# yellofi/SelectiveNet_for_semantic_segmentation_binary

Measured on AMD Instinct MI355X. Metric: train images/sec, SelectiveUNet_B 256x256 bs=128 (global), selective_loss s_lamb=2, higher is better.
Workload: dtype f32; 1 GPU; SelectiveUNet_B train step, global bs=128, 256x256, Adam lr=1e-3, s_lamb=2; model=SelectiveUNet_B, global_batch=128, per_gpu_batch=128, image=256, parallelism=dp1

## Files before the change

### selectivenet_for_semantic_segmentation_binary_amd/csrc/conv3x3.hip

```cpp
#include <cstdlib>

#include "gemm_common.h"

namespace selunet {

constexpr int TH = 16, TW = 16;
constexpr int HHT = TH + 2, HWT = TW + 2;
constexpr int HPIX = HHT * HWT;
constexpr int HTHREADS = 512;
constexpr int A_ROUNDS = (HPIX * 8 + HTHREADS - 1) / HTHREADS;
constexpr int AROWB = 160;
__device__ __forceinline__ int halo_off(int hp, int cc) { return hp * AROWB + ((cc ^ ((hp / HWT) & 1)) << 4); }

template <typename T, int BN, bool ONE_CHUNK>
__global__ void __launch_bounds__(HTHREADS, ONE_CHUNK ? 2 : 1)
conv3x3_halo_kernel(GatherArg g, const T* __restrict__ B, int N, int k_pad, EpiArg ep, int n_tiles, int tiles_x,
                    int tiles_y) {
  constexpr int E = 16 / sizeof(T);
  constexpr int CK = 128 / sizeof(T);
  constexpr int WAVES_N = BN / 64;
  constexpr int WAVES_M = 8 / WAVES_N;
  constexpr int WPIX = (TH * TW) / WAVES_M;
  constexpr int MT = WPIX / 32;
  constexpr int NT = 2;
// ... 133 lines not shown
  b_store(rb_next, 0);
  rb_next = b_load(nsteps > 1 ? 1 : 0);
  __syncthreads();

  if constexpr (ONE_CHUNK) {
#pragma unroll
    for (int t = 0; t < 9; ++t) {
      BRegs rb_far = rb_next;
      if (t + 2 < 9) rb_far = b_load(t + 2);
      mma_step(0, t & 1, t);
      if (t + 1 < 9) b_store(rb_next, (t + 1) & 1);
      __syncthreads();
      rb_next = rb_far;
    }
  } else {
    uint4 ra[A_ROUNDS];
    for (int c = 0; c < nchunks; ++c) {
      const int cn = c + 1 < nchunks ? c + 1 : c;
      int cs = cn * CK;
      const bool s1 = g.nsrc > 1 && cs >= g.src[0].C;
      if (s1) cs -= g.src[0].C;
      const SrcArg sn = pick_src(g, s1 ? 1 : 0);
      float* ssc = Ss + ((c + 1) & 1) * CK;
      float* ssh = Ss + 2 * CK + ((c + 1) & 1) * CK;
      float coef = 0.0f;
#pragma unroll
      for (int t = 0; t < 9; ++t) {
        const int s = c * 9 + t;
        const BRegs rb_far = b_load(s + 2 < nsteps ? s + 2 : nsteps - 1);
        if (t == 0 && sn.scale && tid < 2 * CK) coef = tid < CK ? sn.scale[cs + tid] : sn.shift[cs + tid - CK];
        if (t < A_ROUNDS) {
          int hp, cc;
          a_slot(t, hp, cc);
          ra[t] = *a_ptr(cn, hp, cc);
        }
        mma_step(c & 1, s & 1, t);
        b_store(rb_next, (s + 1) & 1);
        if (t == 1 && sn.scale && tid < 2 * CK) (tid < CK ? ssc[tid] : ssh[tid - CK]) = coef;
        if (t >= AD && t - AD < A_ROUNDS) {
          const int r = t - AD;
          int hp, cc;
          if (a_slot(r, hp, cc)) {
            uint4 v = make_uint4(0, 0, 0, 0);
            if (a_inside(hp)) {
              v = ra[r];
              if (sn.scale) {
                T e[E];
                __builtin_memcpy(e, &v, 16);
#pragma unroll
                for (int j = 0; j < E; ++j) {
                  float f = to_f(e[j]) * ssc[cc * E + j] + ssh[cc * E + j];
                  if (sn.relu) f = fmaxf(f, 0.0f);
                  e[j] = from_f<T>(f);
                }
                __builtin_memcpy(&v, e, 16);
              }
            }
            *reinterpret_cast<uint4*>(As + ((c + 1) & 1) * HPIX * AROWB + halo_off(hp, cc)) = v;
          }
        }
        __syncthreads();
        rb_next = rb_far;
      }
    }
  }

  float* tile = reinterpret_cast<float*>(smem);
  acc_to_lds<MT, NT, BN>(tile, acc, wm * WPIX, wn * 64, lane);
  __syncthreads();
  auto dst = [&](int pix, int c) -> T* {
    const int y = y0 + pix / TW, x = x0 + pix % TW;
    if (y >= g.h || x >= g.w) return nullptr;
    const int64_t m = ((int64_t)img * g.h + y) * g.w + x;
    const int col = n0 + c;
    if (ep.mode == SELUNET_EP_SPLIT)
      return col < ep.split ? reinterpret_cast<T*>(ep.out0) + m * ep.split + col
                            : reinterpret_cast<T*>(ep.out1) + m * (N - ep.split) + (col - ep.split);
    return reinterpret_cast<T*>(ep.out0) + m * N + col;
  };
  auto bias_col = [&](int c) { return n0 + c; };
  lds_tile_store<T, TH * TW, BN, HTHREADS>(tile, tid, dst, ep.bias, bias_col, tile_stats(ep, ptile, n0, N));
}

template <typename T, int BN, bool X2, bool M16 = false, bool TQ = false>
__global__ void __launch_bounds__(HTHREADS, 1)
conv3x3_halo_persist_kernel(GatherArg g, const T* __restrict__ B, int N, int k_pad, EpiArg ep, int n_tiles,
                            int tiles_x, int tiles_y, int ptiles, int gp, const float* __restrict__ wcs,
                            const float* __restrict__ amax0, const float* __restrict__ amax1,
                            unsigned* __restrict__ tq = nullptr) {
  static_assert(!TQ || X2, "tile queue: split-fp16 kernel only");
  static_assert(!X2 || std::is_same<T, float>::value, "split-fp16 form of fp32 operands only");
  static_assert(!M16 || X2, "16x16x32 form: split-fp16 only (the bf16 form lost every A/B, retired in round 6)");
  constexpr int E = 16 / sizeof(T);
  constexpr int CK = 128 / sizeof(T);
  constexpr int WAVES_N = BN / 64;
  constexpr int WAVES_M = 8 / WAVES_N;
  constexpr int WPIX = (TH * TW) / WAVES_M;
  constexpr int MT = WPIX / 32;
  constexpr int NT = 2;
  constexpr int RT = WPIX / 16;
  using AccT = std::conditional_t<M16, f32x4, f32x16>;
  constexpr int AM = M16 ? RT : MT, AN = M16 ? 4 : NT;
  constexpr int WROWB = M16 ? 160 : ROWB;
  constexpr int B_ROUNDS = BN * 8 / HTHREADS;
  static_assert(B_ROUNDS * HTHREADS == BN * 8, "weight tile rows must split evenly over the threads");
  auto halo_load_tap = [](int r) { return r; };
  auto halo_write_tap = [](int r) { return r + 3; };
  static_assert(A_ROUNDS <= 6, "halo slice schedule covers six slices");

  constexpr int SMEM_MAIN = 2 * HPIX * AROWB + 2 * BN * WROWB + 2 * CK * 8;
  constexpr int SMEM_EPI = TH * TW * (BN + 4) * 4;
  __shared__ __attribute__((aligned(16))) unsigned char smem[SMEM_MAIN > SMEM_EPI ? SMEM_MAIN : SMEM_EPI];
  unsigned char* As = smem;
  unsigned char* Bs = smem + 2 * HPIX * AROWB;
  float* Ss = reinterpret_cast<float*>(Bs + 2 * BN * WROWB);

  const int tid = threadIdx.x;
  const int lane = tid & 63, wave = tid >> 6;
  const int wm = wave / WAVES_N, wn = wave % WAVES_N;
  const int half = lane >> 5, l32 = lane & 31;
  const int l16 = lane & 15, kg = lane >> 4;

  const unsigned lb = xcd_remap(blockIdx.x, gridDim.x);
  const int n_tile = lb % n_tiles;
  const int prow = lb / n_tiles;
  const int n0 = n_tile * BN;
  const int nchunks = g.Ctot / CK;
  const int ntl = TQ ? 0 : (prow < ptiles ? (ptiles - prow + gp - 1) / gp : 0);
  __shared__ int tq_slot;
  int pt_cur = 0, pt_next = 0;
  if constexpr (TQ) {
    if (tid == 0) tq_slot = (int)min(atomicAdd(tq + n_tile, 1u), (unsigned)ptiles);
    __syncthreads();
    pt_cur = tq_slot;
  }
  const int csteps = nchunks * 9;
  float xs = 1.0f;
  float cfac[AN] = {};
  if constexpr (X2) {
    float am = amax0 ? amax0[0] : 0.0f;
    if (g.nsrc > 1 && amax1) am = fmaxf(am, amax1[0]);
    float inv;
    xs = x2_scale(am, &inv);
#pragma unroll
    for (int b = 0; b < AN; ++b)
      cfac[b] = wcs[n0 + wn * 64 + (M16 ? b * 16 + l16 : b * 32 + l32)] * inv;
  }
  auto halo_store = [&](int hb, int hp, int cc, uint4 v) __attribute__((always_inline)) {
    unsigned char* base = As + hb * HPIX * AROWB + hp * AROWB;
    if constexpr (X2) {
      float f[4];
      __builtin_memcpy(f, &v, 16);
      f16x4 h, l;
#pragma unroll
      for (int e = 0; e < 4; ++e) {
        _Float16 a, b;
        x2_split(f[e] * xs, a, b);
        h[e] = a;
        l[e] = b;
      }
      const int par = (hp / HWT) & 1;
      *reinterpret_cast<f16x4*>(base + (((cc >> 1) ^ par) << 4) + (cc & 1) * 8) = h;
      *reinterpret_cast<f16x4*>(base + (((4 + (cc >> 1)) ^ par) << 4) + (cc & 1) * 8) = l;
    } else {
      *reinterpret_cast<uint4*>(base + (((cc ^ ((hp / HWT) & 1))) << 4)) = v;
    }
  };

  auto halo_store_prepped = [&](int hb, int hp, int cc, uint4 v) __attribute__((always_inline)) {
    unsigned char* base = As + hb * HPIX * AROWB + hp * AROWB;
    if constexpr (X2) {
      const int par = (hp / HWT) & 1;
      *reinterpret_cast<uint2*>(base + (((cc >> 1) ^ par) << 4) + (cc & 1) * 8) = make_uint2(v.x, v.y);
      *reinterpret_cast<uint2*>(base + (((4 + (cc >> 1)) ^ par) << 4) + (cc & 1) * 8) = make_uint2(v.z, v.w);
    } else {
      *reinterpret_cast<uint4*>(base + (((cc ^ ((hp / HWT) & 1))) << 4)) = v;
    }
  };
  auto tile_xy = [&](int pt_i, int& img, int& y0, int& x0) __attribute__((always_inline)) {
    const unsigned pt = (unsigned)pt_i;
    const unsigned r = pt / (unsigned)tiles_x;
    x0 = (int)(pt - r * (unsigned)tiles_x) * TW;
    const unsigned r2 = r / (unsigned)tiles_y;
    y0 = (int)(r - r2 * (unsigned)tiles_y) * TH;
    img = (int)r2;
  };
  auto a_slot = [&](int round, int& hp, int& cc) -> bool {
    const int hidx = round * HTHREADS + tid;
    hp = min(hidx >> 3, HPIX - 1);
    cc = hidx & 7;
    return hidx < HPIX * 8;
  };
  auto a_inside = [&](int y0, int x0, int hp) -> bool {
    const int hy = hp / HWT, hx = hp - (hp / HWT) * HWT;
    return (unsigned)(y0 - 1 + hy) < (unsigned)g.h && (unsigned)(x0 - 1 + hx) < (unsigned)g.w;
  };
  auto chunk_src = [&](int chunk, int& c) -> SrcArg {
    c = chunk * CK;
    const bool s1 = g.nsrc > 1 && c >= g.src[0].C;
    if (s1) c -= g.src[0].C;
    return pick_src(g, s1 ? 1 : 0);
  };
  auto a_ptr = [&](const SrcArg& sa, int c, int img, int y0, int x0, int hp, int cc) -> const uint4* {
    const int hy = hp / HWT, hx = hp - (hp / HWT) * HWT;
    const int ys = min(max(y0 - 1 + hy, 0), g.h - 1), xs = min(max(x0 - 1 + hx, 0), g.w - 1);
    return reinterpret_cast<const uint4*>(reinterpret_cast<const T*>(sa.data) +
                                          (((int64_t)img * g.h + ys) * g.w + xs) * sa.C + c + cc * E);
  };
  constexpr int XRPIX = 3 * HWT;
  static_assert(!X2 || (A_ROUNDS * 3 == HHT && XRPIX * 8 <= HTHREADS), "three halo rows per round");
  const int xq = tid >> 3, xcc = tid & 7;
  const int xhp = xq < XRPIX ? xq : xq - XRPIX;
  const int xry = (xhp >= HWT) + (xhp >= 2 * HWT), xhx = xhp - xry * HWT;
  const unsigned xpix = (unsigned)(xry * g.w + xhx);
  const unsigned xb_off = (unsigned)(xq * k_pad * 4 + xcc * 16);
  const unsigned xb_rstride = (unsigned)(64 * k_pad * 4);
  auto x_lds = [](int t) __attribute__((always_inline)) {
    const int q = t >> 3, cc = t & 7, hp = q < XRPIX ? q : q - XRPIX;
    const int ry = (hp >= HWT) + (hp >= 2 * HWT);
    return (unsigned)(hp * AROWB + (((cc >> 1) ^ (ry & 1)) << 4) + (cc & 1) * 8);
  };
  const unsigned xlds = x_lds(tid);
  unsigned xtb = 0;
  if constexpr (X2) {
    const int hrem = g.h - (tiles_y - 1) * TH, wrem = g.w - (tiles_x - 1) * TW;
#pragma unroll
    for (int r = 0; r < A_ROUNDS; ++r) {
      const int hy = 3 * r + xry;
      xtb |= (unsigned)((hy == 0) | (hy > hrem) << 6 | (xhx == 0) << 12 | (xhx > wrem) << 18) << r;
// ... 140 lines not shown
#pragma unroll
      for (int ks = 0; ks < 2; ++ks) {
        f16x8 ah[MT], al[MT], bh[NT], bl[NT];
#pragma unroll
        for (int a = 0; a < MT; ++a) {
          const unsigned char* p = a_src + (hrow0[a] + tap_off) * AROWB + ((hsw0[a] ^ dy) & 1) * 16;
          ah[a] = *reinterpret_cast<const f16x8*>(p + ks * 32);
          al[a] = *reinterpret_cast<const f16x8*>(p + (2 + ks) * 32);
        }
#pragma unroll
        for (int b = 0; b < NT; ++b) {
          const unsigned char* p = b_src + (wn * 64 + b * 32 + l32) * ROWB + half * 16;
          bh[b] = *reinterpret_cast<const f16x8*>(p + ks * 32);
          bl[b] = *reinterpret_cast<const f16x8*>(p + (2 + ks) * 32);
        }
#pragma unroll
        for (int a = 0; a < MT; ++a)
#pragma unroll
          for (int b = 0; b < NT; ++b) {
            acc[a][b] = __builtin_amdgcn_mfma_f32_32x32x16_f16(ah[a], bl[b], acc[a][b], 0, 0, 0);
            acc[a][b] = __builtin_amdgcn_mfma_f32_32x32x16_f16(al[a], bh[b], acc[a][b], 0, 0, 0);
            acc[a][b] = __builtin_amdgcn_mfma_f32_32x32x16_f16(ah[a], bh[b], acc[a][b], 0, 0, 0);
          }
      }
    } else {
#pragma unroll
      for (int q = 0; q < 4; ++q) {
        const int boff = q * 32 + half * 16;
        uint4 af[MT], bfr[NT];
#pragma unroll
        for (int a = 0; a < MT; ++a)
          af[a] = *reinterpret_cast<const uint4*>(a_src + (hrow0[a] + tap_off) * AROWB + q * 32 + ((hsw0[a] ^ dy) & 1) * 16);
#pragma unroll
        for (int b = 0; b < NT; ++b)
          bfr[b] = *reinterpret_cast<const uint4*>(b_src + (wn * 64 + b * 32 + l32) * WROWB + boff);
#pragma unroll
        for (int a = 0; a < MT; ++a)
#pragma unroll
          for (int b = 0; b < NT; ++b) Mma<T>::run(acc[a][b], af[a], bfr[b]);
      }
    }
  };
  auto halo_put_global = [&](uint4 v, int r, const SrcArg& sa, int c, int y0, int x0, int hb)
      __attribute__((always_inline)) {
    int hp, cc;
    if (!a_slot(r, hp, cc)) return;
    uint4 o = make_uint4(0, 0, 0, 0);
    if (a_inside(y0, x0, hp)) o = sa.scale ? transform16<T>(v, sa.scale, sa.shift, c + cc * E, sa.relu) : v;
    halo_store(hb, hp, cc, o);
  };

  Geo gc{}, gn{};
  if constexpr (X2) gc = gn = tile_geo(TQ ? pt_cur : prow);
  if (!TQ || pt_cur < ptiles) {
    int c0;
    const SrcArg sa = chunk_src(0, c0);
    uint4 v0[A_ROUNDS];
    if constexpr (X2) {
      const XStage s0 = x_stage(gc, sa, c0);
#pragma unroll
      for (int r = 0; r < A_ROUNDS; ++r) v0[r] = x_load(s0, sa, r);
#pragma unroll
      for (int r = 0; r < A_ROUNDS; ++r) {
        uint4 o = make_uint4(0, 0, 0, 0);
        if (!x_out(s0, r)) o = sa.scale ? transform16<T>(v0[r], sa.scale, sa.shift, c0 + xcc * E, sa.relu) : v0[r];
        x_put(0, r, xlds, x_split4(o));
      }
    } else {
      int img, y0, x0;
      tile_xy(TQ ? pt_cur : prow, img, y0, x0);
#pragma unroll
      for (int r = 0; r < A_ROUNDS; ++r) {
        int hp, cc;
        a_slot(r, hp, cc);
        v0[r] = *a_ptr(sa, c0, img, y0, x0, hp, cc);
      }
#pragma unroll
      for (int r = 0; r < A_ROUNDS; ++r) halo_put_global(v0[r], r, sa, c0, y0, x0, 0);
    }
  }
  BRegs rb_next = b_load(0);
  b_store(rb_next, 0);
  rb_next = b_load(1 % csteps);
  __syncthreads();

  using Acc = std::conditional_t<X2 && BN == 128, float, typename StatAcc<T>::type>;
  static_assert(stats_flush_bytes<BN, HTHREADS, Acc>() <= (int)sizeof(smem), "statistics scratch exceeds LDS");
  Acc s1[8] = {0, 0, 0, 0, 0, 0, 0, 0}, s2[8] = {0, 0, 0, 0, 0, 0, 0, 0}, s3[8] = {0, 0, 0, 0, 0, 0, 0, 0};
  float amx = 0.0f;
  const TileStats ts = tile_stats(ep, TQ ? 0 : prow, n0, N);
  float* tile = reinterpret_cast<float*>(smem);
  uint4 ra[A_ROUNDS];
  int J = 0;
  int S = 0;
  unsigned claimed = 0;
  for (int i = 0; TQ ? pt_cur < ptiles : i < ntl; ++i) {
    int img, y0, x0;
    if constexpr (X2) {
      img = gc.img, y0 = gc.y0, x0 = gc.x0;
      if constexpr (!TQ) gn = i + 1 < ntl ? tile_geo(prow + (i + 1) * gp) : gc;
    } else {
      tile_xy(TQ ? pt_cur : prow + i * gp, img, y0, x0);
    }
    BRegs rb_hold;
    for (int c = 0; c < nchunks; ++c, ++J) {
      if constexpr (TQ) {
        if (c == 1) {
          pt_next = tq_slot;
          gn = pt_next < ptiles ? tile_geo(pt_next) : gc;
        }
      }
      const bool last_c = c + 1 == nchunks;
      const bool has_next = !last_c || (TQ ? pt_next < ptiles : i + 1 < ntl);
      const bool defer = last_c && has_next;
      int nimg = img, ny0 = y0, nx0 = x0;
      if constexpr (!X2) {
        if (defer) tile_xy(TQ ? pt_next : prow + (i + 1) * gp, nimg, ny0, nx0);
      }
      const int nc = !has_next ? c : (last_c ? 0 : c + 1);
      int cs;
      const SrcArg sn = chunk_src(nc, cs);
      XStage sx{};
      if constexpr (X2) sx = x_stage(defer ? gn : gc, sn, cs);
      float* ssc = Ss + ((J + 1) & 1) * CK;
      float* ssh = Ss + 2 * CK + ((J + 1) & 1) * CK;
      float coef = 0.0f;
#pragma unroll
      for (int t = 0; t < 9; ++t) {
        const int st2 = c * 9 + t + 2;
        const BRegs rb_far = b_load(st2 < csteps ? st2 : st2 - csteps);
        if (t == 0 && sn.scale && tid < 2 * CK) coef = tid < CK ? sn.scale[cs + tid] : sn.shift[cs + tid - CK];
#pragma unroll
        for (int r = 0; r < A_ROUNDS; ++r) {
          if (halo_load_tap(r) == t) {
            if constexpr (X2) {
              ra[r] = x_load(sx, sn, r);
            } else {
              int hp, cc;
              a_slot(r, hp, cc);
              ra[r] = *a_ptr(sn, cs, nimg, ny0, nx0, hp, cc);
            }
          }
        }
        if constexpr (TQ) {
          if (c == 0 && t == 0 && tid == 0) claimed = atomicAdd(tq + n_tile, 1u);
        }
        mma_step(J & 1, S & 1, t);
        if constexpr (TQ) {
          if (c == 0 && t == 8 && tid == 0) tq_slot = (int)min(claimed, (unsigned)ptiles);
        }
        if (defer && t == 8) rb_hold = rb_next;
        else b_store(rb_next, (S + 1) & 1);
        if (t == 1 && sn.scale && tid < 2 * CK) (tid < CK ? ssc[tid] : ssh[tid - CK]) = coef;
#pragma unroll
        for (int r = 0; r < A_ROUNDS; ++r) {
          if (halo_write_tap(r) != t) continue;
          if constexpr (X2) {
            uint4 v = ra[r];
#ifndef SELUNET_ABL_RAW_HALO
            if (sn.scale) {
              float e[4];
              __builtin_memcpy(e, &v, 16);
#pragma unroll
              for (int j = 0; j < 4; ++j) {
                float f = e[j] * ssc[xcc * 4 + j] + ssh[xcc * 4 + j];
                if (sn.relu) f = fmaxf(f, 0.0f);
                e[j] = f;
              }
              __builtin_memcpy(&v, e, 16);
            }
            if (x_out(sx, r)) v = make_uint4(0, 0, 0, 0);
#endif
            const uint4 o = x_split4(v);
            if (!defer) x_put((J + 1) & 1, r, xlds, o);
            else ra[r] = o;
            continue;
          }
          int hp, cc;
          if (a_slot(r, hp, cc)) {
            uint4 v = make_uint4(0, 0, 0, 0);
            if (a_inside(ny0, nx0, hp)) {
              v = ra[r];
              if (sn.scale) {
                T e[E];
                __builtin_memcpy(e, &v, 16);
#pragma unroll
                for (int j = 0; j < E; ++j) {
                  float f = to_f(e[j]) * ssc[cc * E + j] + ssh[cc * E + j];
                  if (sn.relu) f = fmaxf(f, 0.0f);
                  e[j] = from_f<T>(f);
                }
                __builtin_memcpy(&v, e, 16);
              }
            }
            if (!defer) {
              halo_store((J + 1) & 1, hp, cc, v);
            } else {
              if constexpr (X2) {
                float f[4];
                __builtin_memcpy(f, &v, 16);
                f16x4 h, l;
#pragma unroll
                for (int e = 0; e < 4; ++e) {
                  _Float16 a, b;
                  x2_split(f[e] * xs, a, b);
                  h[e] = a;
                  l[e] = b;
                }
                __builtin_memcpy(&v.x, &h, 8);
                __builtin_memcpy(&v.z, &l, 8);
              }
              ra[r] = v;
            }
          }
        }
        __syncthreads();
        rb_next = rb_far;
        ++S;
      }
      if (defer) {
      }
    }

    if constexpr (X2) {
#pragma unroll
      for (int a = 0; a < AM; ++a)
#pragma unroll
        for (int b = 0; b < AN; ++b) acc[a][b] *= cfac[b];
    }
    if constexpr (M16) {
#pragma unroll
      for (int a = 0; a < RT; ++a)
#pragma unroll
        for (int b = 0; b < 4; ++b)
#pragma unroll
          for (int i = 0; i < 4; ++i)
            tile[(wm * WPIX + a * 16 + 4 * kg + i) * (BN + 4) + wn * 64 + b * 16 + l16] = acc[a][b][i];
    } else {
      acc_to_lds<MT, NT, BN>(tile, acc, wm * WPIX, wn * 64, lane);
    }
#pragma unroll
    for (int a = 0; a < AM; ++a)
#pragma unroll
      for (int b = 0; b < AN; ++b) acc[a][b] = AccT{};
    __syncthreads();
    auto dst = [&](int pix, int cl) -> T* {
      const int y = y0 + pix / TW, x = x0 + pix % TW;
      if (y >= g.h || x >= g.w) return nullptr;
      const int64_t m = ((int64_t)img * g.h + y) * g.w + x;
      const int col = n0 + cl;
      if (ep.mode == SELUNET_EP_SPLIT)
        return col < ep.split ? reinterpret_cast<T*>(ep.out0) + m * ep.split + col
                              : reinterpret_cast<T*>(ep.out1) + m * (N - ep.split) + (col - ep.split);
      return reinterpret_cast<T*>(ep.out0) + m * N + col;
    };
    auto bias_col = [&](int cl) { return n0 + cl; };
    if constexpr (TQ) {
      TileStats tt = tile_stats(ep, pt_cur, n0, N);
      lds_tile_store_acc<T, TH * TW, BN, HTHREADS>(tile, tid, dst, ep.bias, bias_col, tt, s1, s2, s3, amx);
      tt.amax = nullptr;
      tile_stats_flush<BN, HTHREADS>(tile, tid, tt, s1, s2, s3, 0.0f);
#pragma unroll
      for (int e = 0; e < 8; ++e) s1[e] = s2[e] = s3[e] = 0;
    } else {
      lds_tile_store_acc<T, TH * TW, BN, HTHREADS>(tile, tid, dst, ep.bias, bias_col, ts, s1, s2, s3, amx);
    }
    if (TQ ? pt_next < ptiles : i + 1 < ntl) {
      __syncthreads();
      int tid2 = tid;
      asm volatile("" : "+v"(tid2));
#pragma unroll
      for (int r = 0; r < A_ROUNDS; ++r) {
        if constexpr (X2) {
          x_put(J & 1, r, x_lds(tid2), ra[r]);
        } else {
          const int hidx = r * HTHREADS + tid2;
          if (hidx < HPIX * 8) halo_store_prepped(J & 1, hidx >> 3, hidx & 7, ra[r]);
        }
      }
      b_store(rb_hold, S & 1);
      __syncthreads();
    }
    if constexpr (TQ) pt_cur = pt_next;
    gc = gn;
  }
  if constexpr (TQ) {
    if (ts.amax) block_amax(ts.amax, amx, tile);
    if (tid == 0 && atomicAdd(tq + n_tiles + n_tile, 1u) == (unsigned)gp - 1u) {
      atomicExch(tq + n_tile, 0u);
      atomicExch(tq + n_tiles + n_tile, 0u);
    }
  } else {
    tile_stats_flush<BN, HTHREADS>(tile, tid, ts, s1, s2, s3, amx);
  }
}

constexpr int WINO_STEPS = 12;
__device__ __forceinline__ int wino_row(int hp) {
  const int hy = hp / HWT, hx = hp - hy * HWT;
  return hy * HWT + (hx & 1) * (HWT / 2) + (hx >> 1);
}

template <int BN, int XS>
__global__ void __launch_bounds__(HTHREADS, 1)
conv3x3_wino_persist_kernel(GatherArg g, const float* __restrict__ B, int N, int k_pad, EpiArg ep, int n_tiles,
                            int tiles_x, int tiles_y, int ptiles, int gp) {
  using T = float;
  constexpr int E = 4;
  constexpr int CK = 32;
  constexpr int NT = BN / 64;
  constexpr int STEPS = WINO_STEPS / XS;
  constexpr int BROWS = XS * BN;
  constexpr int B_ROUNDS = BROWS * 8 / HTHREADS;
  static_assert(XS == 1 || XS == 2, "one or two planes per step");
  auto lt = [](int r) { return XS == 1 ? r : r >> 1; };
  static_assert(B_ROUNDS * HTHREADS == BROWS * 8, "weight tile rows must split evenly over the threads");
  static_assert(A_ROUNDS <= 6, "halo slice schedule covers six slices");

  constexpr int SMEM_MAIN = 2 * HPIX * AROWB + 2 * BROWS * ROWB + 2 * CK * 8;
  constexpr int SMEM_EPI = TH * TW * (BN + 4) * 4;
  __shared__ __attribute__((aligned(16))) unsigned char smem[SMEM_MAIN > SMEM_EPI ? SMEM_MAIN : SMEM_EPI];
  unsigned char* As = smem;
  unsigned char* Bs = smem + 2 * HPIX * AROWB;
  float* Ss = reinterpret_cast<float*>(Bs + 2 * BROWS * ROWB);

  const int tid = threadIdx.x;
  const int lane = tid & 63, wave = tid >> 6;
  const int wm = wave >> 1, wn = wave & 1;
  const int half = lane >> 5, l32 = lane & 31;
  const int pair = wm * 32 + l32, py = pair >> 3, px2 = pair & 7;

  const unsigned lb = xcd_remap(blockIdx.x, gridDim.x);
  const int n_tile = lb % n_tiles;
  const int prow = lb / n_tiles;
  const int n0 = n_tile * BN;
  const int ntl = prow < ptiles ? (ptiles - prow + gp - 1) / gp : 0;
  const int nchunks = g.Ctot / CK;
  const int csteps = nchunks * STEPS;

  auto tile_xy = [&](int i, int& img, int& y0, int& x0) __attribute__((always_inline)) {
    const unsigned pt = (unsigned)(prow + i * gp);
    const unsigned r = pt / (unsigned)tiles_x;
    x0 = (int)(pt - r * (unsigned)tiles_x) * TW;
    const unsigned r2 = r / (unsigned)tiles_y;
    y0 = (int)(r - r2 * (unsigned)tiles_y) * TH;
    img = (int)r2;
  };
// ... 1641 lines not shown
```

### selectivenet_for_semantic_segmentation_binary_amd/csrc/gemm_common.h

```cpp
#pragma once

#include <type_traits>

#include "common.h"

namespace selunet {

struct SrcArg {
  const void* data;
  const float* scale;
  const float* shift;
  int C;
  int relu;
  int layout;
  int pad;
};

struct GatherArg {
  int n, h, w;
  int taps;
  int nsrc;
  int Ctot;
  int hs, ws;
  int K;
// ... 218 lines not shown
      sc[e] = ts.bnb.scale[col + e];
      sh[e] = ts.bnb.shift[col + e];
      mu[e] = ts.bnb.mean[col + e];
      is[e] = ts.bnb.invstd[col + e];
    }
  }
  __builtin_amdgcn_s_waitcnt(0x0F70);
  constexpr bool WIDE = !std::is_same<Acc, float>::value;
  float tw1[WIDE ? 8 : 1] = {}, tw2[WIDE ? 8 : 1] = {}, tw3[WIDE ? 8 : 1] = {};
  float* t1 = WIDE ? tw1 : reinterpret_cast<float*>(s1);
  float* t2 = WIDE ? tw2 : reinterpret_cast<float*>(s2);
  float* t3 = WIDE ? tw3 : reinterpret_cast<float*>(s3);
  constexpr int NR = TR / RS;
  constexpr int YB = NR < (TC >= 128 ? 4 : 2) ? NR : (TC >= 128 ? 4 : 2);
  static_assert(TR % RS == 0 && NR % YB == 0, "epilogue rows must split evenly over the threads");
#pragma unroll 1
  for (int rb = 0; rb < NR; rb += YB) {
  T yb[YB][8];
  if (do_bn) {
#pragma unroll
    for (int j = 0; j < YB; ++j) {
      const T* p = dst(r0 + (rb + j) * RS, col);
      if (p == nullptr) continue;
      const T* yp = reinterpret_cast<const T*>(ts.bnb.y) + (p - reinterpret_cast<const T*>(ts.out0));
      if constexpr (sizeof(T) == 2) {
        const uint4 u = *reinterpret_cast<const uint4*>(yp);
        __builtin_memcpy(yb[j], &u, 16);
      } else {
        const f32x4 a = *reinterpret_cast<const f32x4*>(yp), b = *reinterpret_cast<const f32x4*>(yp + 4);
        __builtin_memcpy(yb[j], &a, 16);
        __builtin_memcpy(yb[j] + 4, &b, 16);
      }
    }
  }
#pragma unroll
  for (int j = 0; j < YB; ++j) {
    const int row = r0 + (rb + j) * RS;
    T* p = dst(row, col);
    if (p == nullptr) continue;
    const f32x4 lo = *reinterpret_cast<const f32x4*>(tile + row * (TC + 4) + col);
    const f32x4 hi = *reinterpret_cast<const f32x4*>(tile + row * (TC + 4) + col + 4);
    float v[8] = {lo[0], lo[1], lo[2], lo[3], hi[0], hi[1], hi[2], hi[3]};
    if (do_st) {
#pragma unroll
      for (int e = 0; e < 8; ++e) {
        const float d = v[e] - cen[e];
        t1[e] += d;
        t2[e] += d * d;
      }
    }
#pragma unroll
    for (int e = 0; e < 8; ++e) v[e] += bv[e];
    T o[8];
#pragma unroll
    for (int e = 0; e < 8; ++e) o[e] = from_f<T>(v[e]);
    if (ts.amax) {
#pragma unroll
      for (int e = 0; e < 8; ++e) am = fmaxf(am, fabsf(to_f(o[e])));
    }
    if constexpr (sizeof(T) == 2) {
      uint4 u;
      __builtin_memcpy(&u, o, 16);
      *reinterpret_cast<uint4*>(p) = u;
    } else {
      *reinterpret_cast<f32x4*>(p) = f32x4{v[0], v[1], v[2], v[3]};
      *reinterpret_cast<f32x4*>(p + 4) = f32x4{v[4], v[5], v[6], v[7]};
    }
    if (do_cs) {
#pragma unroll
      for (int e = 0; e < 8; ++e) t1[e] += to_f(o[e]);
    }
    if (do_bn) {
#pragma unroll
      for (int e = 0; e < 8; ++e) {
        const float y = to_f(yb[j][e]);
        const float da = y * sc[e] + sh[e] > 0.0f ? to_f(o[e]) : 0.0f;
        const float xh = (y - mu[e]) * is[e];
        t1[e] += da;
        t2[e] += da * xh;
        t3[e] += xh;
      }
    }
  }
  }
  if constexpr (WIDE) {
#pragma unroll
    for (int e = 0; e < 8; ++e) {
      s1[e] += (Acc)t1[e];
      s2[e] += (Acc)t2[e];
      s3[e] += (Acc)t3[e];
    }
  }
}

template <int TC, int NTHREADS, typename Acc>
constexpr int stats_flush_bytes() { return (NTHREADS / (TC / 8)) * TC * 3 * (int)sizeof(Acc); }

template <int TC, int NTHREADS, typename Acc>
__device__ __forceinline__ void tile_stats_flush(float* red_f, int tid, const TileStats& ts, const Acc (&s1)[8],
                                                 const Acc (&s2)[8], const Acc (&s3)[8], float am) {
  constexpr int CC = TC / 8;
  constexpr int RS = NTHREADS / CC;
  Acc* red = reinterpret_cast<Acc*>(red_f);
  const int cc = tid % CC, r0 = tid / CC;
  const int col = cc * 8;
  const bool do_st = ts.stats != nullptr;
  const bool do_bn = ts.bnb.slab != nullptr;
  const int nst = do_bn ? 3 : (do_st ? 2 : 1);
  if (do_st || ts.colsum != nullptr || do_bn) {
    __syncthreads();
#pragma unroll
    for (int e = 0; e < 8; ++e) {
      red[(r0 * TC + col + e) * 3 + 0] = s1[e];
      red[(r0 * TC + col + e) * 3 + 1] = s2[e];
      red[(r0 * TC + col + e) * 3 + 2] = s3[e];
    }
    __syncthreads();
    for (int i = tid; i < TC * nst; i += NTHREADS) {
      const int c = i % TC, k = i / TC;
      Acc a = 0;
      for (int r = 0; r < RS; ++r) a += red[(r * TC + c) * 3 + k];
      if (do_bn) ts.bnb.slab[k * ts.ld + c] = a;
      else if (do_st) ts.stats[k * ts.ld + c] = a;
      else if (ts.gcol0 + c < ts.colsum_cols) ts.colsum[c] = a;
    }
  }
  if (ts.amax) block_amax(ts.amax, am, red_f);
}

template <typename T, int TR, int TC, int NTHREADS, typename Dst, typename BiasCol>
__device__ __forceinline__ void lds_tile_store(float* tile, int tid, Dst&& dst, const float* bias, BiasCol&& bias_col,
                                               const TileStats& ts) {
  float s1[8] = {0, 0, 0, 0, 0, 0, 0, 0}, s2[8] = {0, 0, 0, 0, 0, 0, 0, 0}, s3[8] = {0, 0, 0, 0, 0, 0, 0, 0};
  float am = 0.0f;
  lds_tile_store_acc<T, TR, TC, NTHREADS>(tile, tid, dst, bias, bias_col, ts, s1, s2, s3, am);
  tile_stats_flush<TC, NTHREADS>(tile, tid, ts, s1, s2, s3, am);
}

int make_gather(const selunet_gather* a, int dtype, GatherArg& g, int vec_elems);

bool conv3x3_halo_eligible(const GatherArg& g, int N, int dtype);
int64_t conv3x3_halo_tiles(const GatherArg& g);
int64_t conv3x3_halo_stats_rows(const GatherArg& g, int N, int dtype);
bool conv3x3_halo_one_chunk(const GatherArg& g, int dtype);
bool conv3x3_halo_persistent(const GatherArg& g, int dtype);
int conv3x3_halo_launch(const GatherArg& g, const void* b, int N, int k_pad, const EpiArg& ep, int dtype,
                        hipStream_t st);
bool conv3x3_wino_shape_ok(int h, int w, int c_in, int c_src0, int n_cols);
bool conv3x3_wgrad_wino_eligible(const GatherArg& p, const GatherArg& q, int dtype);
int64_t conv3x3_wgrad_wino_splits(const GatherArg& p, const GatherArg& q);
int conv3x3_wgrad_wino_launch(const GatherArg& p, const GatherArg& q, float* ws, int ldw, hipStream_t st);
bool conv3x3_wino_eligible(const GatherArg& g, int N);
bool conv3x3_bn128(int N, const EpiArg& ep, int split_mult);
int conv3x3_wino_launch(const GatherArg& g, const float* u, int N, const EpiArg& ep, hipStream_t st);
bool conv3x3_x2_shape_ok(int h, int w, int c_in, int c_src0, int n_cols);
bool conv3x3_x2_eligible(const GatherArg& g, int N);
int conv3x3_x2_launch(const GatherArg& g, const float* w, int N, const EpiArg& ep, const float* amax0,
                      const float* amax1, hipStream_t st);
bool convt_x2_eligible(const GatherArg& g, int N, const EpiArg& e);
int convt_dgrad_x2_ntb(const GatherArg& g, int N);
int64_t convt_dgrad_x2_rows(const GatherArg& g, int N);
bool convt_dgrad_x2_eligible(const GatherArg& g, int N, const EpiArg& e);
int convt_dgrad_x2_launch(const GatherArg& g, const float* w, int N, const EpiArg& e, const float* amax_src,
                          hipStream_t st);
bool convt_ring_dgrad_operand_ok(const GatherArg& g, int N);
int64_t convt_ring_rows(const GatherArg& g, int N);
// ... 56 lines not shown
```

Baseline: 1415 images/s.

## Stage epilogue coefficients in LDS and prefetch BN input rows before tile barrier

For the split-fp16 persistent 3x3 conv kernel, per-column epilogue coefficients (bias, stats center, BN scale/shift/mean/invstd, weight column scale) are loaded once into an LDS region instead of being refetched per tile. The BN-backward y rows are issued as global loads before the post-accumulator barrier and software-pipelined across epilogue rows. Row addressing is precomputed with a validity mask. This aims to hide global latency in the epilogue, at the cost of extra LDS, more registers for in-flight y rows, and a new tunable depth.

```diff
diff --git a/selectivenet_for_semantic_segmentation_binary_amd/csrc/conv3x3.hip b/selectivenet_for_semantic_segmentation_binary_amd/csrc/conv3x3.hip
--- a/selectivenet_for_semantic_segmentation_binary_amd/csrc/conv3x3.hip
+++ b/selectivenet_for_semantic_segmentation_binary_amd/csrc/conv3x3.hip
@@ -239,6 +239,12 @@
   lds_tile_store<T, TH * TW, BN, HTHREADS>(tile, tid, dst, ep.bias, bias_col, tile_stats(ep, ptile, n0, N));
 }
 
+#ifndef SELUNET_EPI_YB128
+#define SELUNET_EPI_YB128 5
+#endif
+#ifndef SELUNET_EPI_YB64
+#define SELUNET_EPI_YB64 4
+#endif
 template <typename T, int BN, bool X2, bool M16 = false, bool TQ = false>
 __global__ void __launch_bounds__(HTHREADS, 1)
 conv3x3_halo_persist_kernel(GatherArg g, const T* __restrict__ B, int N, int k_pad, EpiArg ep, int n_tiles,
@@ -267,7 +273,10 @@
 
   constexpr int SMEM_MAIN = 2 * HPIX * AROWB + 2 * BN * WROWB + 2 * CK * 8;
   constexpr int SMEM_EPI = TH * TW * (BN + 4) * 4;
-  __shared__ __attribute__((aligned(16))) unsigned char smem[SMEM_MAIN > SMEM_EPI ? SMEM_MAIN : SMEM_EPI];
+  constexpr int SMEM_UNION = SMEM_MAIN > SMEM_EPI ? SMEM_MAIN : SMEM_EPI;
+  constexpr int SMEM_COEF = X2 ? epi_coef_bytes<BN>() + BN * 4 : 0;
+  static_assert(SMEM_UNION % 16 == 0 && SMEM_UNION + SMEM_COEF + 16 <= 160 * 1024, "LDS budget of one workgroup per CU");
+  __shared__ __attribute__((aligned(16))) unsigned char smem[SMEM_UNION + SMEM_COEF];
   unsigned char* As = smem;
   unsigned char* Bs = smem + 2 * HPIX * AROWB;
   float* Ss = reinterpret_cast<float*>(Bs + 2 * BN * WROWB);
@@ -293,15 +302,13 @@
   }
   const int csteps = nchunks * 9;
   float xs = 1.0f;
-  float cfac[AN] = {};
+  float* ecoef = reinterpret_cast<float*>(smem + SMEM_UNION);
   if constexpr (X2) {
     float am = amax0 ? amax0[0] : 0.0f;
     if (g.nsrc > 1 && amax1) am = fmaxf(am, amax1[0]);
     float inv;
     xs = x2_scale(am, &inv);
-#pragma unroll
-    for (int b = 0; b < AN; ++b)
-      cfac[b] = wcs[n0 + wn * 64 + (M16 ? b * 16 + l16 : b * 32 + l32)] * inv;
+    for (int c = tid; c < BN; c += HTHREADS) ecoef[EPI_COEF_ROWS * BN + c] = wcs[n0 + c] * inv;
   }
   auto halo_store = [&](int hb, int hp, int cc, uint4 v) __attribute__((always_inline)) {
     unsigned char* base = As + hb * HPIX * AROWB + hp * AROWB;
@@ -608,10 +615,11 @@
   BRegs rb_next = b_load(0);
   b_store(rb_next, 0);
   rb_next = b_load(1 % csteps);
+  if constexpr (X2) epi_coef_fill<BN, HTHREADS>(ecoef, tid, ep, n0);
   __syncthreads();
 
   using Acc = std::conditional_t<X2 && BN == 128, float, typename StatAcc<T>::type>;
-  static_assert(stats_flush_bytes<BN, HTHREADS, Acc>() <= (int)sizeof(smem), "statistics scratch exceeds LDS");
+  static_assert(stats_flush_bytes<BN, HTHREADS, Acc>() <= SMEM_UNION, "statistics scratch exceeds LDS");
   Acc s1[8] = {0, 0, 0, 0, 0, 0, 0, 0}, s2[8] = {0, 0, 0, 0, 0, 0, 0, 0}, s3[8] = {0, 0, 0, 0, 0, 0, 0, 0};
   float amx = 0.0f;
   const TileStats ts = tile_stats(ep, TQ ? 0 : prow, n0, N);
@@ -749,6 +757,9 @@
     }
 
     if constexpr (X2) {
+      float cfac[AN];
+#pragma unroll
+      for (int b = 0; b < AN; ++b) cfac[b] = ecoef[EPI_COEF_ROWS * BN + wn * 64 + (M16 ? b * 16 + l16 : b * 32 + l32)];
 #pragma unroll
       for (int a = 0; a < AM; ++a)
 #pragma unroll
@@ -765,30 +776,68 @@
     } else {
       acc_to_lds<MT, NT, BN>(tile, acc, wm * WPIX, wn * 64, lane);
     }
-#pragma unroll
-    for (int a = 0; a < AM; ++a)
-#pragma unroll
-      for (int b = 0; b < AN; ++b) acc[a][b] = AccT{};
-    __syncthreads();
-    auto dst = [&](int pix, int cl) -> T* {
-      const int y = y0 + pix / TW, x = x0 + pix % TW;
-      if (y >= g.h || x >= g.w) return nullptr;
-      const int64_t m = ((int64_t)img * g.h + y) * g.w + x;
-      const int col = n0 + cl;
-      if (ep.mode == SELUNET_EP_SPLIT)
-        return col < ep.split ? reinterpret_cast<T*>(ep.out0) + m * ep.split + col
-                              : reinterpret_cast<T*>(ep.out1) + m * (N - ep.split) + (col - ep.split);
-      return reinterpret_cast<T*>(ep.out0) + m * N + col;
-    };
-    auto bias_col = [&](int cl) { return n0 + cl; };
-    if constexpr (TQ) {
-      TileStats tt = tile_stats(ep, pt_cur, n0, N);
-      lds_tile_store_acc<T, TH * TW, BN, HTHREADS>(tile, tid, dst, ep.bias, bias_col, tt, s1, s2, s3, amx);
-      tt.amax = nullptr;
-      tile_stats_flush<BN, HTHREADS>(tile, tid, tt, s1, s2, s3, 0.0f);
-#pragma unroll
-      for (int e = 0; e < 8; ++e) s1[e] = s2[e] = s3[e] = 0;
+    if constexpr (!X2) {
+#pragma unroll
+      for (int a = 0; a < AM; ++a)
+#pragma unroll
+        for (int b = 0; b < AN; ++b) acc[a][b] = AccT{};
+    }
+    if constexpr (X2) {
+      constexpr int ERS = HTHREADS / (BN / 8);
+      constexpr int ENR = epi_rows<TH * TW, BN, HTHREADS>();
+      static_assert(ERS % TW == 0, "a thread's epilogue rows keep their tile column");
+      constexpr int EYB = BN >= 128 ? SELUNET_EPI_YB128 : SELUNET_EPI_YB64;
+      auto erows = [&](int r0, int cl) __attribute__((always_inline)) {
+        const int py = r0 / TW, px = r0 % TW;
+        const int col = n0 + cl;
+        int gw = g.w;
+        asm volatile("" : "+s"(gw));
+        float* base = reinterpret_cast<float*>(ep.out0) + col;
+        int64_t ld = N;
+        if (ep.mode == SELUNET_EP_SPLIT) {
+          ld = col < ep.split ? ep.split : N - ep.split;
+          if (col >= ep.split) base = reinterpret_cast<float*>(ep.out1) + (col - ep.split);
+        }
+        EpiRows er;
+        er.safe = base + gc.pix * ld;
+        er.p = er.safe + (int64_t)(py * gw + px) * ld;
+        er.stride = (int64_t)((ERS / TW) * gw) * ld;
+        er.ok = 0;
+        if (gc.x0 + px < g.w) {
+#pragma unroll
+          for (int j = 0; j < ENR; ++j) er.ok |= (unsigned)(gc.y0 + py + j * (ERS / TW) < g.h) << j;
+        }
+        return er;
+      };
+      TileStats tt = TQ ? tile_stats(ep, pt_cur, n0, N) : ts;
+      f32x4 yb[EYB][2];
+      __builtin_amdgcn_sched_barrier(0);
+      lds_tile_y_issue<TH * TW, BN, HTHREADS, EYB>(tid, erows, tt, yb);
+      __syncthreads();
+      lds_tile_store_res<TH * TW, BN, HTHREADS, EYB>(tile, ecoef, tid, erows, yb, tt, s1, s2, s3, amx);
+      if constexpr (TQ) {
+        tt.amax = nullptr;
+        tile_stats_flush<BN, HTHREADS>(tile, tid, tt, s1, s2, s3, 0.0f);
+#pragma unroll
+        for (int e = 0; e < 8; ++e) s1[e] = s2[e] = s3[e] = 0;
+      }
+#pragma unroll
+      for (int a = 0; a < AM; ++a)
+#pragma unroll
+        for (int b = 0; b < AN; ++b) acc[a][b] = AccT{};
     } else {
+      __syncthreads();
+      auto dst = [&](int pix, int cl) -> T* {
+        const int y = y0 + pix / TW, x = x0 + pix % TW;
+        if (y >= g.h || x >= g.w) return nullptr;
+        const int64_t m = ((int64_t)img * g.h + y) * g.w + x;
+        const int col = n0 + cl;
+        if (ep.mode == SELUNET_EP_SPLIT)
+          return col < ep.split ? reinterpret_cast<T*>(ep.out0) + m * ep.split + col
+                                : reinterpret_cast<T*>(ep.out1) + m * (N - ep.split) + (col - ep.split);
+        return reinterpret_cast<T*>(ep.out0) + m * N + col;
+      };
+      auto bias_col = [&](int cl) { return n0 + cl; };
       lds_tile_store_acc<T, TH * TW, BN, HTHREADS>(tile, tid, dst, ep.bias, bias_col, ts, s1, s2, s3, amx);
     }
     if (TQ ? pt_next < ptiles : i + 1 < ntl) {
diff --git a/selectivenet_for_semantic_segmentation_binary_amd/csrc/gemm_common.h b/selectivenet_for_semantic_segmentation_binary_amd/csrc/gemm_common.h
--- a/selectivenet_for_semantic_segmentation_binary_amd/csrc/gemm_common.h
+++ b/selectivenet_for_semantic_segmentation_binary_amd/csrc/gemm_common.h
@@ -324,6 +324,161 @@
       }
     }
   }
+  }
+  if constexpr (WIDE) {
+#pragma unroll
+    for (int e = 0; e < 8; ++e) {
+      s1[e] += (Acc)t1[e];
+      s2[e] += (Acc)t2[e];
+      s3[e] += (Acc)t3[e];
+    }
+  }
+}
+
+constexpr int EPI_COEF_ROWS = 6;
+template <int TC>
+constexpr int epi_coef_bytes() { return EPI_COEF_ROWS * TC * 4; }
+
+template <int TC, int NTHREADS>
+__device__ __forceinline__ void epi_coef_fill(float* coef, int tid, const EpiArg& ep, int n0) {
+  const bool bn = ep.bnb.slab != nullptr;
+  for (int i = tid; i < EPI_COEF_ROWS * TC; i += NTHREADS) {
+    const int k = i / TC, c = i - k * TC;
+    const float* src = k == 0   ? ep.bias
+                       : k == 1 ? (ep.stats ? ep.stats_center : nullptr)
+                       : !bn    ? nullptr
+                       : k == 2 ? ep.bnb.scale
+                       : k == 3 ? ep.bnb.shift
+                       : k == 4 ? ep.bnb.mean
+                                : ep.bnb.invstd;
+    coef[i] = src ? src[n0 + c] : 0.0f;
+  }
+}
+
+struct EpiRows {
+  float* p;
+  float* safe;
+  int64_t stride;
+  unsigned ok;
+};
+
+template <int TR, int TC, int NTHREADS>
+constexpr int epi_rows() { return TR / (NTHREADS / (TC / 8)); }
+
+__device__ __forceinline__ int64_t epi_y_offset(const TileStats& ts) {
+  const float* y = reinterpret_cast<const float*>(ts.bnb.y);
+  asm volatile("" : "+s"(y));
+  return y - reinterpret_cast<const float*>(ts.out0);
+}
+
+__device__ __forceinline__ void epi_y_load(const EpiRows& er, int j, int64_t yoff, f32x4 (&y)[2]) {
+  const float* yp = ((er.ok >> j) & 1u ? er.p + j * er.stride : er.safe) + yoff;
+  y[0] = *reinterpret_cast<const f32x4*>(yp);
+  y[1] = *reinterpret_cast<const f32x4*>(yp + 4);
+}
+
+template <int TR, int TC, int NTHREADS, int YB, typename Rows>
+__device__ __forceinline__ void lds_tile_y_issue(int tid, Rows&& rows, const TileStats& ts, f32x4 (&yb)[YB][2]) {
+  constexpr int CC = TC / 8;
+  static_assert(YB >= 1 && YB <= epi_rows<TR, TC, NTHREADS>(), "y rows in flight");
+  asm volatile("" : "+v"(tid));
+  const EpiRows er = rows(tid / CC, (tid % CC) * 8);
+#ifndef SELUNET_ABL_EPI_NOY
+  if (ts.bnb.slab != nullptr) {
+    const int64_t yoff = epi_y_offset(ts);
+#pragma unroll
+    for (int j = 0; j < YB; ++j) epi_y_load(er, j, yoff, yb[j]);
+  }
+#endif
+}
+
+template <int TR, int TC, int NTHREADS, int YB, typename Rows, typename Acc>
+__device__ __forceinline__ void lds_tile_store_res(const float* tile, const float* coef, int tid, Rows&& rows,
+                                                   const f32x4 (&yb)[YB][2], const TileStats& ts, Acc (&s1)[8], Acc (&s2)[8], Acc (&s3)[8],
+                                                   float& am) {
+  constexpr int CC = TC / 8;
+  constexpr int RS = NTHREADS / CC;
+  constexpr int NR = epi_rows<TR, TC, NTHREADS>();
+  static_assert(TR % RS == 0 && NR <= 32, "epilogue rows must split evenly over the threads");
+#ifdef SELUNET_ABL_EPI_NOSTORE
+  return;
+#endif
+  asm volatile("" : "+v"(tid));
+  const int cc = tid % CC, r0 = tid / CC;
+  const int col = cc * 8;
+  const bool do_st = ts.stats != nullptr;
+  const bool do_cs = ts.colsum != nullptr && ts.gcol0 + col < ts.colsum_cols;
+  const bool do_bn = ts.bnb.slab != nullptr;
+  const EpiRows er = rows(r0, col);
+  auto coef8 = [&](int k, float (&c)[8]) __attribute__((always_inline)) {
+    const f32x4 lo = *reinterpret_cast<const f32x4*>(coef + k * TC + col);
+    const f32x4 hi = *reinterpret_cast<const f32x4*>(coef + k * TC + col + 4);
+#pragma unroll
+    for (int e = 0; e < 4; ++e) c[e] = lo[e], c[4 + e] = hi[e];
+  };
+  const int64_t yoff = epi_y_offset(ts);
+  float bv[8], cen[8] = {}, sc[8], sh[8], mu[8], is[8];
+  coef8(0, bv);
+  if (do_st) coef8(1, cen);
+  if (do_bn) {
+    coef8(2, sc);
+    coef8(3, sh);
+    coef8(4, mu);
+    coef8(5, is);
+  }
+  constexpr bool WIDE = !std::is_same<Acc, float>::value;
+  float tw1[WIDE ? 8 : 1] = {}, tw2[WIDE ? 8 : 1] = {}, tw3[WIDE ? 8 : 1] = {};
+  float* t1 = WIDE ? tw1 : reinterpret_cast<float*>(s1);
+  float* t2 = WIDE ? tw2 : reinterpret_cast<float*>(s2);
+  float* t3 = WIDE ? tw3 : reinterpret_cast<float*>(s3);
+  f32x4 late[NR > YB ? NR - YB : 1][2];
+#pragma unroll
+  for (int j = 0; j < NR; ++j) {
+#ifndef SELUNET_ABL_EPI_NOY
+    if (do_bn && j >= 1 && j - 1 + YB < NR) epi_y_load(er, j - 1 + YB, yoff, late[j - 1]);
+#endif
+    if (!((er.ok >> j) & 1u)) continue;
+    const int row = r0 + j * RS;
+    float* p = er.p + j * er.stride;
+    const f32x4 lo = *reinterpret_cast<const f32x4*>(tile + row * (TC + 4) + col);
+    const f32x4 hi = *reinterpret_cast<const f32x4*>(tile + row * (TC + 4) + col + 4);
+    float v[8] = {lo[0], lo[1], lo[2], lo[3], hi[0], hi[1], hi[2], hi[3]};
+    if (do_st) {
+#pragma unroll
+      for (int e = 0; e < 8; ++e) {
+        const float d = v[e] - cen[e];
+        t1[e] += d;
+        t2[e] += d * d;
+      }
+    }
+#pragma unroll
+    for (int e = 0; e < 8; ++e) v[e] += bv[e];
+    if (ts.amax) {
+#pragma unroll
+      for (int e = 0; e < 8; ++e) am = fmaxf(am, fabsf(v[e]));
+    }
+    *reinterpret_cast<f32x4*>(p) = f32x4{v[0], v[1], v[2], v[3]};
+    *reinterpret_cast<f32x4*>(p + 4) = f32x4{v[4], v[5], v[6], v[7]};
+    if (do_cs) {
+#pragma unroll
+      for (int e = 0; e < 8; ++e) t1[e] += v[e];
+    }
+    if (do_bn) {
+#pragma unroll
+      for (int e = 0; e < 8; ++e) {
+#ifdef SELUNET_ABL_EPI_NOY
+        const float y = v[e];
+#else
+        const float y = (j < YB ? yb[j < YB ? j : 0] : late[j < YB ? 0 : j - YB])[e >> 2][e & 3];
+#endif
+        const float da = y * sc[e] + sh[e] > 0.0f ? v[e] : 0.0f;
+        const float xh = (y - mu[e]) * is[e];
+        t1[e] += da;
+        t2[e] += da * xh;
+        t3[e] += xh;
+      }
+    }
+    __builtin_amdgcn_sched_barrier(0);
   }
   if constexpr (WIDE) {
 #pragma unroll
```

New measurement: 1422 images/s, median of 6. About the same (+0.5%).
